# JacekNaruniec/LiveScan3D

Measured on AMD Instinct MI355X. Metric: fused frames/s (N x 512x424 depth -> merged cloud), higher is better.
Workload: dtype f32

## Files before the change

livescan3d_amd/csrc/radial.hip:

```cpp
#include "fusion_shared.hpp"

namespace {


struct RadialParams { float cx, cy, fx, fy, r2, r4, r6, pad; };

__device__ __forceinline__ int f2i_x86(float v)
{
    return (v > -2147483904.0f && v < 2147483648.0f) ? (int)v : (int)0x80000000;
}

__global__ __launch_bounds__(kThreads) void radial_warp_kernel(const FrameDesc *frames, const TileDesc *tiles, const RadialParams *rp,
                                                               const unsigned short *depth, unsigned int *winner, int tiles_per_tick,
                                                               long long tick_pix_stride)
{
    const int tick = blockIdx.x / tiles_per_tick;
    const int tile = blockIdx.x - tick * tiles_per_tick;
    const TileDesc td = tiles[tile];
    const FrameDesc fd = frames[td.frame];
    const RadialParams P = rp[td.frame];
    const unsigned short *dep = depth + tick * tick_pix_stride + fd.depth_off;
    unsigned int *win = winner + tick * tick_pix_stride + fd.depth_off;
    const int p0 = (tile - fd.tile_start) * kTile;
    for (int i = threadIdx.x; i < kTile; i += kThreads) {
        const int p = p0 + i;
        if (p >= fd.npix) break;
        if (dep[p] == 0) continue;
        const int y = p / fd.w, x = p - y * fd.w;
        const float u = ((float)x - P.cx) / P.fx;
        const float v = ((float)y - P.cy) / P.fy;
        const float r = u * u + v * v;
        const float d = 1 - P.r2 * r - P.r4 * r * r - P.r6 * r * r * r;
        const int x_corr = f2i_x86(u * d * P.fx + P.cx);
        const int y_corr = f2i_x86(v * d * P.fy + P.cy);
        if (x_corr >= 0 && y_corr >= 0 && x_corr < fd.w && y_corr < fd.h)
            atomicMax(&win[x_corr + (long long)y_corr * fd.w], (unsigned int)p + 1u);
    }
}

__global__ __launch_bounds__(kThreads) void radial_gather_kernel(const FrameDesc *frames, const TileDesc *tiles, const unsigned short *depth,
                                                                 const unsigned char *rgb, const unsigned int *winner,
                                                                 unsigned short *map_copy, unsigned char *colors_copy, int tiles_per_tick,
                                                                 long long tick_pix_stride)
{
    const int tick = blockIdx.x / tiles_per_tick;
    const int tile = blockIdx.x - tick * tiles_per_tick;
    const TileDesc td = tiles[tile];
    const FrameDesc fd = frames[td.frame];
    const long long fb = tick * tick_pix_stride + fd.depth_off;
    const int p0 = (tile - fd.tile_start) * kTile;
    for (int i = threadIdx.x; i < kTile; i += kThreads) {
        const int p = p0 + i;
        if (p >= fd.npix) break;
        const unsigned int wsrc = winner[fb + p];
        unsigned short d = 0;
        unsigned char c0 = 0, c1 = 0, c2 = 0;
        if (wsrc) {
            const long long s = fb + (long long)(wsrc - 1u);
            d = depth[s];
            c0 = rgb[3 * s]; c1 = rgb[3 * s + 1]; c2 = rgb[3 * s + 2];
        }
        map_copy[fb + p] = d;
        colors_copy[3 * (fb + p)] = c0;
        colors_copy[3 * (fb + p) + 1] = c1;
        colors_copy[3 * (fb + p) + 2] = c2;
    }
}

__global__ __launch_bounds__(kThreads) void radial_cand_fill_kernel(const FrameDesc *frames, const TileDesc *tiles, const RadialParams *rp,
                                                                    unsigned int *count, unsigned int *cand, int *overflow)
{
    const int tile = blockIdx.x;
    const TileDesc td = tiles[tile];
    const FrameDesc fd = frames[td.frame];
    const RadialParams P = rp[td.frame];
    const int p0 = (tile - fd.tile_start) * kTile;
    for (int i = threadIdx.x; i < kTile; i += kThreads) {
        const int p = p0 + i;
        if (p >= fd.npix) break;
        const int y = p / fd.w, x = p - y * fd.w;
        const float u = ((float)x - P.cx) / P.fx;
        const float v = ((float)y - P.cy) / P.fy;
        const float r = u * u + v * v;
        const float d = 1 - P.r2 * r - P.r4 * r * r - P.r6 * r * r * r;
        const int x_corr = f2i_x86(u * d * P.fx + P.cx);
        const int y_corr = f2i_x86(v * d * P.fy + P.cy);
        if (x_corr >= 0 && y_corr >= 0 && x_corr < fd.w && y_corr < fd.h) {
            const long long dst = fd.depth_off + x_corr + (long long)y_corr * fd.w;
            const unsigned int slot = atomicAdd(&count[dst], 1u);
            if (slot < 4) cand[4 * dst + slot] = (unsigned int)p + 1u;
            else atomicOr(overflow, 1);
        }
    }
}

__global__ __launch_bounds__(kThreads) void radial_cand_sort_kernel(uint4 *cand, long long n)
{
    const long long i = (long long)blockIdx.x * kThreads + threadIdx.x;
    if (i >= n) return;
    uint4 c = cand[i];
    auto cswap = [](unsigned int &a, unsigned int &b) { const unsigned int hi = max(a, b), lo = min(a, b); a = hi; b = lo; };
    cswap(c.x, c.y); cswap(c.z, c.w); cswap(c.x, c.z); cswap(c.y, c.w); cswap(c.y, c.z);
    cand[i] = c;
}

template <int ELEM, typename T>
__device__ __forceinline__ void store_tile_run(T *dst, const T *lds, int lead, int n)
{
    static_assert(sizeof(T) == ELEM, "element size");
    const int end = lead + n;
    const int c0 = lead ? 1 : 0, c1 = end >> 4;
    uint4 *g16 = reinterpret_cast<uint4 *>(reinterpret_cast<unsigned char *>(dst) - lead);
    const uint4 *l16 = reinterpret_cast<const uint4 *>(lds);
    for (int j = c0 + (int)threadIdx.x; j < c1; j += kThreads) g16[j] = l16[j];
    const int head = lead ? min(n, 16 - lead) : 0;
    const int tail0 = max(head, 16 * c1 - lead);
    const int t = (int)threadIdx.x * ELEM;
    if (t < head) dst[threadIdx.x] = lds[lead / ELEM + threadIdx.x];
    if (tail0 + t < n) dst[tail0 / ELEM + threadIdx.x] = lds[(lead + tail0) / ELEM + threadIdx.x];
}

constexpr unsigned int kWide = 0xFFFFFFFFu;

__global__ __launch_bounds__(kThreads) void radial_cand_pack_kernel(const FrameDesc *frames, const TileDesc *tiles, const uint4 *cand,
                                                                    unsigned int *ctab)
{
    const int tile = blockIdx.x;
    const TileDesc td = tiles[tile];
    const FrameDesc fd = frames[td.frame];
    const int p0 = (tile - fd.tile_start) * kTile;
    for (int i = threadIdx.x; i < kTile; i += kThreads) {
        const int p = p0 + i;
        if (p >= fd.npix) break;
        const uint4 c = cand[fd.depth_off + p];
        auto enc = [&](unsigned int src, unsigned int &code) {
            code = 0;
            if (!src) return true;
            const int rel = (int)(src - 1u) - p;
            if (rel < -32767 || rel > 32767) return false;
            code = (unsigned int)(rel + 32768);
            return true;
        };
        unsigned int c0, c1;
        const bool ok0 = enc(c.x, c0), ok1 = enc(c.y, c1);
        ctab[fd.depth_off + p] = (ok0 && ok1 && c.z == 0) ? (c0 | (c1 << 16)) : kWide;
    }
}

typedef unsigned int u32_ua __attribute__((aligned(1)));
typedef unsigned short u16_ua __attribute__((aligned(1)));
typedef unsigned long long u64_ua __attribute__((aligned(1)));

struct WarpSrc {
    const unsigned short *depth;
    const unsigned char *rgb;
    const unsigned int *ctab;
    const uint4 *cand;
    long long last_px;
};


constexpr unsigned int kRsrcWord3 = 0x00027000u;
constexpr unsigned int kNowhere = 0xFFFFFFF0u;

template <int K, bool SPEC = false>
__device__ __forceinline__ void gather_batch(const WarpSrc &S, long long fb, long long doff, int npix, int pv, const int (&p)[K], const bool (&in)[K],
                                             unsigned int (&d)[K], unsigned int (&rgb)[K])
{
    (void)pv;
    const __amdgpu_buffer_rsrc_t tab = __builtin_amdgcn_make_buffer_rsrc(const_cast<unsigned int *>(S.ctab + doff), 0, 4 * npix, kRsrcWord3);
    const __amdgpu_buffer_rsrc_t dep = __builtin_amdgcn_make_buffer_rsrc(const_cast<unsigned short *>(S.depth + fb), 0, 2 * npix, kRsrcWord3);
    const __amdgpu_buffer_rsrc_t col = __builtin_amdgcn_make_buffer_rsrc(const_cast<unsigned char *>(S.rgb + 3 * fb), 0, 3 * npix, kRsrcWord3);
    const unsigned int last = (unsigned int)npix - 1u;
    auto colour = [&](unsigned int q, bool real) {
        const unsigned int adj = q == last ? 1u : 0u;
        const unsigned int v = __builtin_amdgcn_raw_buffer_load_b32(col, real ? 3u * q - adj : kNowhere, 0, 0);
        return (v >> (8u * adj)) & 0x00FFFFFFu;
    };
    unsigned int e[K];
#pragma unroll
    for (int k = 0; k < K; k++) e[k] = __builtin_amdgcn_raw_buffer_load_b32(tab, in[k] ? 4u * (unsigned int)p[k] : kNowhere, 0, 0);
    unsigned int s0[K], s1[K], d0[K], d1[K], c0[K];
    bool any_wide = false;
#pragma unroll
    for (int k = 0; k < K; k++) {
        const unsigned int a0 = e[k] & 0xFFFFu, a1 = e[k] >> 16;
        const bool wide = e[k] == kWide;
        any_wide |= wide;
        const bool v0 = a0 != 0 && !wide, v1 = a1 != 0 && !wide;
        s0[k] = (unsigned int)p[k] + a0 - 32768u;
        s1[k] = (unsigned int)p[k] + a1 - 32768u;
        d0[k] = __builtin_amdgcn_raw_buffer_load_b16(dep, v0 ? 2u * s0[k] : kNowhere, 0, 0);
        d1[k] = __builtin_amdgcn_raw_buffer_load_b16(dep, v1 ? 2u * s1[k] : kNowhere, 0, 0);
        if (SPEC) c0[k] = colour(s0[k], v0);
    }
    bool second = false;
#pragma unroll
    for (int k = 0; k < K; k++) {
        const unsigned int src = d0[k] ? s0[k] : s1[k];
        d[k] = d0[k] ? d0[k] : d1[k];
        if (SPEC) {
            rgb[k] = d0[k] ? c0[k] : 0u;
            second |= !d0[k] && d1[k];
        } else {
            rgb[k] = colour(src, d[k] != 0);
        }
    }
    if (SPEC && __any(second)) {
#pragma unroll
        for (int k = 0; k < K; k++) {
            const bool need = !d0[k] && d1[k];
            const unsigned int v = colour(s1[k], need);
            if (need) rgb[k] = v;
        }
    }
    if (__any(any_wide)) {
        const unsigned short *gdep = S.depth + fb;
#pragma unroll
        for (int k = 0; k < K; k++) {
            if (e[k] == kWide) {
                const uint4 c = S.cand[doff + p[k]];
                const unsigned int cs[4] = {c.x, c.y, c.z, c.w};
                int sw = -1;
                unsigned int dd = 0;
#pragma unroll
                for (int j = 0; j < 4; j++) {
                    if (sw < 0 && cs[j]) {
                        const unsigned int v = gdep[cs[j] - 1u];
                        if (v) { sw = (int)(cs[j] - 1u); dd = v; }
                    }
                }
                d[k] = dd;
                rgb[k] = colour((unsigned int)(sw >= 0 ? sw : 0), sw >= 0);
            }
        }
    }
}

__device__ __forceinline__ unsigned int one_pixel_colour(const WarpSrc &S, long long fb, unsigned int depth)
{
    const unsigned char *px = S.rgb + 3 * fb;
    return depth ? ((unsigned int)px[0] | ((unsigned int)px[1] << 8) | ((unsigned int)px[2] << 16)) : 0u;
}

__global__ __launch_bounds__(kThreads) void radial_gather_pack_kernel(const FrameDesc *__restrict__ frames, const TileDesc *__restrict__ tiles,
                                                                      const WarpSrc S, unsigned short *__restrict__ map_copy,
                                                                      unsigned char *__restrict__ colors_copy, int tiles_per_tick, long long tick_pix_stride)
{
    const int tick = blockIdx.x / tiles_per_tick;
    const int tile = blockIdx.x - tick * tiles_per_tick;
    const TileDesc td = tiles[tile];
    const FrameDesc fd = frames[td.frame];
    const long long fb = tick * tick_pix_stride + fd.depth_off;
    const int p0 = (tile - fd.tile_start) * kTile;
    __shared__ alignas(16) unsigned short s_d[kTile + 8];
    __shared__ alignas(16) unsigned char s_c[3 * kTile + 16];
    unsigned short *gd = map_copy + fb + p0;
    unsigned char *gc = colors_copy + 3 * (fb + p0);
    const int lead_d = (int)(reinterpret_cast<uintptr_t>(gd) & 15), lead_c = (int)(reinterpret_cast<uintptr_t>(gc) & 15);
    constexpr int kFly = 4;
    for (int i0 = threadIdx.x; i0 < kTile; i0 += kFly * kThreads) {
        int p[kFly];
        bool in[kFly];
#pragma unroll
        for (int k = 0; k < kFly; k++) {
            p[k] = p0 + i0 + k * kThreads;
            in[k] = i0 + k * kThreads < kTile && p[k] < fd.npix;
        }
        unsigned int d[kFly], c[kFly];
        gather_batch<kFly>(S, fb, fd.depth_off, fd.npix, p0, p, in, d, c);
#pragma unroll
        for (int k = 0; k < kFly; k++) {
            if (!in[k]) continue;
            const int i = i0 + k * kThreads;
            s_d[lead_d / 2 + i] = (unsigned short)d[k];
            unsigned char *c3 = s_c + lead_c + 3 * i;
            c3[0] = (unsigned char)c[k];
            c3[1] = (unsigned char)(c[k] >> 8);
            c3[2] = (unsigned char)(c[k] >> 16);
        }
    }
    if (fd.npix == 1 && threadIdx.x == 0) {
        const unsigned int c1 = one_pixel_colour(S, fb, s_d[lead_d / 2]);
        unsigned char *c3 = s_c + lead_c;
        c3[0] = (unsigned char)c1;
        c3[1] = (unsigned char)(c1 >> 8);
        c3[2] = (unsigned char)(c1 >> 16);
    }
    __syncthreads();
    const int n_px = min(kTile, fd.npix - p0);
    store_tile_run<2>(gd, s_d, lead_d, 2 * n_px);
    store_tile_run<1>(gc, s_c, lead_c, 3 * n_px);
}

constexpr int kRing = 32;

struct RingChunk { unsigned int d[4]; unsigned int c[8]; };

__device__ __forceinline__ void ring_load_chunk(const unsigned short *map, const unsigned char *col, int w, int h, int row, int chunk,
                                                RingChunk &reg)
{
    const bool row_ok = row >= 0 && row < h;
    if ((w & 7) == 0) {
        uint4 dv = make_uint4(0, 0, 0, 0);
// ... 11 lines not shown
            const int b = 3 * j;
            const unsigned int lo = cw[b >> 2], hi = cw[(b >> 2) + 1 < 6 ? (b >> 2) + 1 : 5];
            reg.c[j] = __funnelshift_r(lo, hi, (b & 3) * 8) & 0x00FFFFFFu;
        }
        return;
    }
#pragma unroll
    for (int j = 0; j < 8; j++) {
        const int c0 = chunk * 8 + j;
        unsigned int dv = 0, cv = 0;
        if (row_ok && c0 >= 0 && c0 < w) {
            const long long p = (long long)row * w + c0;
            dv = map[p];
            cv = col[3 * p] | (col[3 * p + 1] << 8) | (col[3 * p + 2] << 16);
        }
        if (j & 1) reg.d[j >> 1] |= dv << 16;
        else reg.d[j >> 1] = dv;
        reg.c[j] = cv;
    }
}

__device__ __forceinline__ void ring_store_chunk(unsigned short *dring_row, unsigned int *cring_row, int chunk, const RingChunk &reg)
{
    const int s0 = (chunk * 8) & (kRing - 1);
    unsigned int *dd = reinterpret_cast<unsigned int *>(dring_row + s0);
#pragma unroll
    for (int j = 0; j < 4; j++) dd[j] = reg.d[j];
#pragma unroll
    for (int j = 0; j < 8; j++) cring_row[s0 + j] = reg.c[j];
}

struct RingFeed {
    int ring, row;
    RingChunk p0, p1;
};

__global__ __launch_bounds__(768) void radial_close_kernel(const FrameDesc *frames, int n_frames, unsigned short *map_copy,
                                                            unsigned char *colors_copy, long long tick_pix_stride)
{
    extern __shared__ unsigned int ring_mem[];
    const int rows = blockDim.x;
    unsigned int *cring = ring_mem;
    unsigned short *dring = reinterpret_cast<unsigned short *>(ring_mem + (rows + 2) * kRing);
    const int tick = blockIdx.x / n_frames;
    const int f = blockIdx.x - tick * n_frames;
    const FrameDesc fd = frames[f];
    const int w = fd.w, h = fd.h;
    unsigned short *map = map_copy + tick * tick_pix_stride + fd.depth_off;
    unsigned char *col = colors_copy + 3 * (tick * tick_pix_stride + fd.depth_off);
    const int r = threadIdx.x;
    for (int band0 = 1; band0 < h - 1; band0 += rows) {
        const int y = band0 + r;
        const bool has_a = y <= h - 1;
        const bool has_b = (r == 0) || (r == rows - 1);
        RingFeed A, B;
        A.ring = r + 1; A.row = y;
        B.ring = r == 0 ? 0 : rows + 1; B.row = r == 0 ? band0 - 1 : y + 1;
        const int x_start = 1 - 2 * r;
        auto top_chunk = [](int x0) { return (x0 + 18) >> 3; };
        __syncthreads();
        {
            const int P = top_chunk(x_start);
            if (has_a) {
                for (int c = P - 3; c <= P; c++) {
                    ring_load_chunk(map, col, w, h, A.row, c, A.p0);
                    ring_store_chunk(dring + A.ring * kRing, cring + A.ring * kRing, c, A.p0);
                }
                ring_load_chunk(map, col, w, h, A.row, P + 1, A.p0);
                ring_load_chunk(map, col, w, h, A.row, P + 2, A.p1);
            }
            if (has_b) {
                for (int c = P - 3; c <= P; c++) {
                    ring_load_chunk(map, col, w, h, B.row, c, B.p0);
                    ring_store_chunk(dring + B.ring * kRing, cring + B.ring * kRing, c, B.p0);
                }
                ring_load_chunk(map, col, w, h, B.row, P + 1, B.p0);
                ring_load_chunk(map, col, w, h, B.row, P + 2, B.p1);
            }
        }
        __syncthreads();
        const unsigned short *d_up = dring + r * kRing, *d_below = dring + (r + 2) * kRing;
        unsigned short *d_mine = dring + (r + 1) * kRing;
        const unsigned int *c_up = cring + r * kRing, *c_below = cring + (r + 2) * kRing;
        unsigned int *c_mine = cring + (r + 1) * kRing;
        const int steps = (w - 2) + 2 * (rows - 1);
        for (int t = 0; t < steps; t++) {
            const int x = x_start + t;
            if (t > 0 && (t & 15) == 0) {
                const int P = top_chunk(x);
                if (has_a) {
                    ring_store_chunk(dring + A.ring * kRing, cring + A.ring * kRing, P - 1, A.p0);
                    ring_store_chunk(dring + A.ring * kRing, cring + A.ring * kRing, P, A.p1);
                    ring_load_chunk(map, col, w, h, A.row, P + 1, A.p0);
                    ring_load_chunk(map, col, w, h, A.row, P + 2, A.p1);
                }
                if (has_b) {
                    ring_store_chunk(dring + B.ring * kRing, cring + B.ring * kRing, P - 1, B.p0);
                    ring_store_chunk(dring + B.ring * kRing, cring + B.ring * kRing, P, B.p1);
                    ring_load_chunk(map, col, w, h, B.row, P + 1, B.p0);
                    ring_load_chunk(map, col, w, h, B.row, P + 2, B.p1);
                }
                __builtin_amdgcn_fence(__ATOMIC_RELEASE, "workgroup", "local");
                __builtin_amdgcn_s_barrier();
                __builtin_amdgcn_fence(__ATOMIC_ACQUIRE, "workgroup", "local");
            }
            if (y < h - 1 && x >= 1 && x < w - 1 && d_mine[x & (kRing - 1)] == 0) {
                const int xm = (x - 1) & (kRing - 1), x0 = x & (kRing - 1), xp = (x + 1) & (kRing - 1);
                const int nb[8] = {d_up[xm], d_up[x0], d_up[xp], d_mine[xm], d_mine[xp], d_below[xm], d_below[x0], d_below[xp]};
                int n = 0, sum = 0, prev_val = -1;
                unsigned int accepted = 0;
#pragma unroll
                for (int i = 0; i < 8; i++) {
                    const bool ok = (nb[i] > 0) & ((prev_val == -1) | (abs(nb[i] - prev_val) < 30));
                    prev_val = ok ? nb[i] : prev_val;
                    n += ok ? 1 : 0;
                    sum += ok ? nb[i] : 0;
                    accepted |= (ok ? 1u : 0u) << i;
                }
                if (n > 4) {
                    const unsigned int nc[8] = {c_up[xm], c_up[x0], c_up[xp], c_mine[xm], c_mine[xp], c_below[xm], c_below[x0], c_below[xp]};
                    int sR = 0, sG = 0, sB = 0;
#pragma unroll
                    for (int i = 0; i < 8; i++) {
                        const unsigned int c = (accepted >> i) & 1u ? nc[i] : 0u;
                        sR += c & 0xFF; sG += (c >> 8) & 0xFF; sB += (c >> 16) & 0xFF;
                    }
                    const float rn = 1.0f / (float)n;
                    auto div_n = [&](int v) {
                        int q = (int)((float)v * rn);
                        const int r = v - q * n;
                        q += r >= n ? 1 : 0;
                        q -= r < 0 ? 1 : 0;
                        return (unsigned int)q;
                    };
                    const unsigned int fd_ = div_n(sum);
                    const unsigned int fR = div_n(sR), fG = div_n(sG), fB = div_n(sB);
                    d_mine[x0] = (unsigned short)fd_;
                    c_mine[x0] = fR | (fG << 8) | (fB << 16);
                    const long long pos = x + (long long)y * w;
                    map[pos] = (unsigned short)fd_;
                    col[pos * 3] = (unsigned char)fR;
                    col[pos * 3 + 1] = (unsigned char)fG;
                    col[pos * 3 + 2] = (unsigned char)fB;
                }
            }
            __builtin_amdgcn_fence(__ATOMIC_RELEASE, "workgroup", "local");
            __builtin_amdgcn_s_barrier();
            __builtin_amdgcn_fence(__ATOMIC_ACQUIRE, "workgroup", "local");
        }
    }
}


__device__ __forceinline__ void accept_chain(const int (&nb)[8], int &n, int &sum, unsigned int &accepted)
{
    n = 0;
    sum = 0;
    accepted = 0;
    int prev_val = -1;
#pragma unroll
    for (int i = 0; i < 8; i++) {
        const bool ok = (nb[i] > 0) & ((prev_val == -1) | (abs(nb[i] - prev_val) < 30));
        prev_val = ok ? nb[i] : prev_val;
        n += ok ? 1 : 0;
        sum += ok ? nb[i] : 0;
        accepted |= (ok ? 1u : 0u) << i;
    }
}

__device__ __forceinline__ unsigned int div_small(int v, int n)
{
    const float rn = 1.0f / (float)n;
    int q = (int)((float)v * rn);
    const int r = v - q * n;
    q += r >= n ? 1 : 0;
    q -= r < 0 ? 1 : 0;
    return (unsigned int)q;
}

__device__ __forceinline__ unsigned int average_colour(const unsigned int (&nc)[8], unsigned int accepted, int n)
{
    int sR = 0, sG = 0, sB = 0;
#pragma unroll
    for (int i = 0; i < 8; i++) {
        const unsigned int c = (accepted >> i) & 1u ? nc[i] : 0u;
        sR += c & 0xFF; sG += (c >> 8) & 0xFF; sB += (c >> 16) & 0xFF;
    }
    return div_small(sR, n) | (div_small(sG, n) << 8) | (div_small(sB, n) << 16);
}

constexpr int kDx[8] = {-1, 0, 1, -1, 1, -1, 0, 1}, kDy[8] = {-1, -1, -1, 0, 0, 1, 1, 1};

__device__ __forceinline__ int wave_reserve(int *counter, int mine)
{
    const int lane = threadIdx.x & 63;
    const int incl = wave_inclusive_scan(mine, lane);
    const int total = __shfl(incl, 63, 64);
    int base = 0;
    if (total > 0) {
        if (lane == 0) base = atomicAdd(counter, total);
        base = __shfl(base, 0, 64);
    }
    return base + incl - mine;
}

constexpr int kCntStride = 32;
#ifndef LSN_BAND_THREADS
#define LSN_BAND_THREADS 256
#endif
constexpr int kBandThreads = LSN_BAND_THREADS;

struct BandDesc { int frame, y0; };

__device__ __forceinline__ long long hole_base_bit(const FrameDesc &fd, int f) { return ((fd.depth_off + 63) & ~63ll) + 64ll * f; }

struct BandArgs {
    const FrameDesc *frames;
    const BandDesc *bands;
    WarpSrc src;
    unsigned short *out_d;
    unsigned char *out_c;
    unsigned char *holes;
    unsigned int *work;
    int *work_cnt;
    int bands_per_tick, n_frames, rows;
    long long tick_pix_stride, holes_tick_bytes;
};

constexpr int kBandList = 8192;

__host__ __device__ inline int band_list_entries(int rows, int w)
{
    const int all = rows * w;
    return all <= kBandList ? all : (kBandList > w ? kBandList : w);
}

__host__ __device__ inline int band_lds_bytes(int rows, int w)
{
    const int band_px = (rows + 2) * w;
    return 16 + ((2 * band_px + 15) & ~15) + 16 + ((3 * band_px + 15) & ~15) + ((2 * band_list_entries(rows, w) + 15) & ~15) + 16;
}

__device__ __forceinline__ void store_band_run(unsigned char *dst, const unsigned char *lds, int n)
{
    const int lead = (int)(reinterpret_cast<uintptr_t>(dst) & 15);
    const int head = lead ? min(n, 16 - lead) : 0;
    const int chunks = (n - head) >> 4;
    const uint4 *l16 = reinterpret_cast<const uint4 *>(lds + head);
    uint4 *g16 = reinterpret_cast<uint4 *>(dst + head);
    for (int j = threadIdx.x; j < chunks; j += kBandThreads) g16[j] = l16[j];
    const int tail0 = head + 16 * chunks;
    if ((int)threadIdx.x < head) dst[threadIdx.x] = lds[threadIdx.x];
    if (tail0 + (int)threadIdx.x < n) dst[tail0 + threadIdx.x] = lds[tail0 + threadIdx.x];
}

__device__ __forceinline__ unsigned int pk_min1(unsigned int x)
{
    unsigned int r;
    asm("v_pk_min_u16 %0, %1, %2" : "=v"(r) : "v"(x), "v"(0x00010001u));
    return r;
}

template <bool GATHER, bool VEC>
__global__ __launch_bounds__(kBandThreads) void radial_band_kernel(const BandArgs a)
{
    extern __shared__ __attribute__((aligned(16))) unsigned char smem[];
    const int tid = threadIdx.x;
    const int tick = blockIdx.x / a.bands_per_tick;
    const int band = blockIdx.x - tick * a.bands_per_tick;
    const BandDesc bd = a.bands[band];
    const FrameDesc fd = a.frames[bd.frame];
    const int w = fd.w, h = fd.h, y0 = bd.y0;
    const int nrows = min(a.rows, h - y0);
    const long long fb = tick * a.tick_pix_stride + fd.depth_off;
    const int tf = tick * a.n_frames + bd.frame;
    const int band_px = (a.rows + 2) * w;
    unsigned short *gd = a.out_d + fb + (long long)y0 * w;
    unsigned char *gc = a.out_c + 3 * (fb + (long long)y0 * w);
    const int lead_d = (int)((reinterpret_cast<uintptr_t>(gd) - 2 * (uintptr_t)w) & 15);
    const int lead_c = (int)((reinterpret_cast<uintptr_t>(gc) - 3 * (uintptr_t)w) & 15);
    const int off_c = 16 + ((2 * band_px + 15) & ~15);
    const int off_l = off_c + 16 + ((3 * band_px + 15) & ~15);
    unsigned short *s_d = reinterpret_cast<unsigned short *>(smem + lead_d);
    unsigned char *s_c = smem + off_c + lead_c;
    unsigned short *s_list = reinterpret_cast<unsigned short *>(smem + off_l);
    const int list_entries = band_list_entries(a.rows, w);
    int *s_n = reinterpret_cast<int *>(smem + off_l + ((2 * list_entries + 15) & ~15));
    const int pl0 = (y0 - 1) * w;
    const int lo = pl0 < 0 ? -pl0 : 0;
    const int hi = min((nrows + 2) * w, fd.npix - pl0);

    if (GATHER) {
#ifndef LSN_BAND_FLY
#define LSN_BAND_FLY 8
#endif
        constexpr int kFly = LSN_BAND_FLY;
        for (int i0 = lo + tid; i0 < hi; i0 += kFly * kBandThreads) {
            int p[kFly];
            bool in[kFly];
#pragma unroll
            for (int k = 0; k < kFly; k++) {
                p[k] = pl0 + i0 + k * kBandThreads;
                in[k] = i0 + k * kBandThreads < hi;
            }
            unsigned int d[kFly], c[kFly];
#ifndef LSN_BAND_SPEC
#define LSN_BAND_SPEC false
#endif
            gather_batch<kFly, LSN_BAND_SPEC>(a.src, fb, fd.depth_off, fd.npix, pl0 + lo, p, in, d, c);
#pragma unroll
            for (int k = 0; k < kFly; k++) {
                if (!in[k]) continue;
                const int i = i0 + k * kBandThreads;
                s_d[i] = (unsigned short)d[k];
                unsigned char *c3 = s_c + 3 * i;
                c3[0] = (unsigned char)c[k];
                c3[1] = (unsigned char)(c[k] >> 8);
                c3[2] = (unsigned char)(c[k] >> 16);
            }
        }
        if (fd.npix == 1 && tid == 0) {
            const unsigned int c1 = one_pixel_colour(a.src, fb, s_d[lo]);
            unsigned char *c3 = s_c + 3 * lo;
            c3[0] = (unsigned char)c1;
            c3[1] = (unsigned char)(c1 >> 8);
            c3[2] = (unsigned char)(c1 >> 16);
        }
    } else if (VEC) {
        const unsigned short *sd = a.src.depth + fb + pl0;
        const unsigned char *sc = a.src.rgb + 3 * (fb + pl0);
        for (int i = lo + 8 * tid; i < hi; i += 8 * kBandThreads) {
            *reinterpret_cast<uint4 *>(s_d + i) = *reinterpret_cast<const uint4 *>(sd + i);
            const uint2 *cp = reinterpret_cast<const uint2 *>(sc + 3 * i);
            uint2 *lp = reinterpret_cast<uint2 *>(s_c + 3 * i);
            const uint2 c0 = cp[0], c1 = cp[1], c2 = cp[2];
            lp[0] = c0; lp[1] = c1; lp[2] = c2;
        }
    } else {
        const unsigned short *sd = a.src.depth + fb + pl0;
        const unsigned char *sc = a.src.rgb + 3 * (fb + pl0);
        for (int i = lo + tid; i < hi; i += kBandThreads) {
            s_d[i] = sd[i];
            s_c[3 * i] = sc[3 * i];
            s_c[3 * i + 1] = sc[3 * i + 1];
            s_c[3 * i + 2] = sc[3 * i + 2];
        }
    }
    __syncthreads();

    store_band_run(reinterpret_cast<unsigned char *>(gd), reinterpret_cast<const unsigned char *>(s_d + w), 2 * nrows * w);
    store_band_run(gc, s_c + 3 * w, 3 * nrows * w);

    const long long hole_bit0 = hole_base_bit(fd, bd.frame);
    unsigned char *holes = a.holes + tick * a.holes_tick_bytes;
    unsigned int *work = a.work + 2 * fb;
    int *work_cnt = a.work_cnt + kCntStride * tf;
    const int rows_per_chunk = max(1, list_entries / w);
    for (int r0 = 0; r0 < nrows; r0 += rows_per_chunk) {
        const int r1 = min(nrows, r0 + rows_per_chunk);
        __syncthreads();
        if (tid == 0) *s_n = 0;
        __syncthreads();
        if (VEC) {
            const int gw = w >> 3, ngroups = (r1 - r0) * gw;
            for (int g0 = 0; g0 < ngroups; g0 += kBandThreads) {
                const int g = g0 + tid;
                unsigned int cb = 0;
                int li = 0;
                if (g < ngroups) {
                    const int r = r0 + g / gw, x0 = (g % gw) << 3, y = y0 + r;
                    li = (r + 1) * w + x0;
                    unsigned int m[3];
#pragma unroll
                    for (int rr = 0; rr < 3; rr++) {
                        const unsigned short *row = s_d + li + (rr - 1) * w;
                        const uint4 c = *reinterpret_cast<const uint4 *>(row);
                        const unsigned int left = x0 > 0 ? row[-1] : 0u, right = x0 + 8 < w ? row[8] : 0u;
                        const unsigned int p0 = pk_min1(c.x) | (pk_min1(c.y) << 2), p1 = pk_min1(c.z) | (pk_min1(c.w) << 2);
                        const unsigned int q0 = (p0 | (p0 >> 15)) & 0xFu, q1 = (p1 | (p1 >> 15)) & 0xFu;
                        m[rr] = (left ? 1u : 0u) | ((q0 | (q1 << 4)) << 1) | (right ? (1u << 9) : 0u);
                    }
                    const unsigned int hb = ~(m[1] >> 1) & 0xFFu;
                    holes[(hole_bit0 + (long long)y * w + x0) >> 3] = (unsigned char)hb;
                    if (y >= 1 && y < h - 1) {
                        const unsigned int n0 = m[0], n1 = m[0] >> 1, n2 = m[0] >> 2, n3 = m[1], n4 = m[1] >> 2, n5 = m[2], n6 = m[2] >> 1, n7 = m[2] >> 2;
                        const unsigned int s1 = n0 ^ n1 ^ n2, c1 = (n0 & n1) | (n2 & (n0 ^ n1));
                        const unsigned int s2 = n5 ^ n6 ^ n7, c2 = (n5 & n6) | (n7 & (n5 ^ n6));
                        const unsigned int s3 = n3 ^ n4, c3 = n3 & n4;
                        const unsigned int t0 = s1 ^ s2 ^ s3, d1 = (s1 & s2) | (s3 & (s1 ^ s2));
                        const unsigned int u0 = c1 ^ c2 ^ c3, e1 = (c1 & c2) | (c3 & (c1 ^ c2));
                        const unsigned int v0 = u0 ^ d1, f1 = u0 & d1;
                        const unsigned int w0 = e1 ^ f1, g1 = e1 & f1;
                        unsigned int inside = 0xFFu;
                        if (x0 == 0) inside &= ~1u;
                        if (x0 + 8 == w) inside &= ~0x80u;
                        cb = (g1 | (w0 & (v0 | t0))) & hb & inside;
                    }
                }
                int slot = wave_reserve(s_n, __popc(cb));
#pragma unroll
                for (int k = 0; k < 8; k++)
                    if ((cb >> k) & 1u) s_list[slot++] = (unsigned short)(li + k);
            }
        } else {
            unsigned int *hw = reinterpret_cast<unsigned int *>(holes);
            const int n_px = (r1 - r0) * w;
            for (int i0 = 0; i0 < n_px; i0 += kBandThreads) {
                const int i = r0 * w + i0 + tid;
                bool cand = false;
                const int li = w + i;
                if (i0 + tid < n_px && s_d[li] == 0) {
                    const int r = i / w, x = i - r * w, y = y0 + r;
                    const long long bit = hole_bit0 + (long long)y * w + x;
                    atomicOr(&hw[bit >> 5], 1u << (bit & 31));
                    if (y >= 1 && y < h - 1 && x >= 1 && x < w - 1) {
                        int nv = 0;
#pragma unroll
                        for (int j = 0; j < 8; j++) nv += s_d[li + kDy[j] * w + kDx[j]] != 0 ? 1 : 0;
                        cand = nv >= 5;
                    }
                }
                const int slot = wave_reserve(s_n, cand ? 1 : 0);
                if (cand) s_list[slot] = (unsigned short)li;
            }
        }
        __syncthreads();
        const int n_cand = *s_n;
        for (int i0 = 0; i0 < n_cand; i0 += kBandThreads) {
            const int i = i0 + tid;
            if (i0 + (tid & ~63) >= n_cand) continue;
            unsigned int succ = 0;
            int x = 0, y = 0;
            if (i < n_cand) {
                const int q = (int)s_list[i];
                int nb[8];
#pragma unroll
                for (int j = 0; j < 8; j++) nb[j] = s_d[q + kDy[j] * w + kDx[j]];
                int n, sum;
                unsigned int accepted;
                accept_chain(nb, n, sum, accepted);
                if (n > 4) {
                    unsigned int nc[8];
#pragma unroll
                    for (int j = 0; j < 8; j++) {
                        const unsigned char *c3 = s_c + 3 * (q + kDy[j] * w + kDx[j]);
                        nc[j] = (accepted >> j) & 1u ? ((unsigned int)c3[0] | ((unsigned int)c3[1] << 8) | ((unsigned int)c3[2] << 16)) : 0u;
                    }
                    const unsigned int rgb = average_colour(nc, accepted, n);
                    const long long pos = fb + pl0 + q;
                    a.out_d[pos] = (unsigned short)div_small(sum, n);
                    a.out_c[3 * pos] = (unsigned char)rgb;
                    a.out_c[3 * pos + 1] = (unsigned char)(rgb >> 8);
                    a.out_c[3 * pos + 2] = (unsigned char)(rgb >> 16);
                    int yl = (int)((float)q * fd.inv_w);
                    x = q - yl * w;
                    if (x < 0) { yl--; x += w; }
                    if (x >= w) { yl++; x -= w; }
                    y = y0 - 1 + yl;
                    const bool below = y + 1 < h - 1;
                    succ = ((nb[4] == 0 && x + 1 < w - 1) ? 1u : 0u) | ((nb[5] == 0 && x - 1 >= 1 && below) ? 2u : 0u) |
                           ((nb[6] == 0 && below) ? 4u : 0u) | ((nb[7] == 0 && x + 1 < w - 1 && below) ? 8u : 0u);
                }
            }
            int slot = wave_reserve(work_cnt, __popc(succ));
#pragma unroll
            for (int sidx = 0; sidx < 4; sidx++) {
                if ((succ >> sidx) & 1u) {
                    const int j = 4 + sidx;
                    if (slot < 2 * fd.npix) work[slot] = (unsigned int)((y + kDy[j]) * w + x + kDx[j]);
                    slot++;
                }
            }
        }
    }
}

#ifndef LSN_FIX_THREADS
#define LSN_FIX_THREADS 256
#endif
constexpr int kFixThreads = LSN_FIX_THREADS;
constexpr int kFixList = 8192;

struct FixArgs {
    const FrameDesc *frames;
    unsigned short *out_d;
    unsigned char *out_c;
    const unsigned char *holes;
    const unsigned int *work;
    int *work_cnt;
    int n_frames, list_cap;
    int n_tf, cnt_index;
    long long tick_pix_stride, holes_tick_bytes;
};

__device__ __forceinline__ bool fix_pixel(unsigned short *out_d, unsigned char *out_c, const unsigned char *holes, long long bit0, int p, int w, int h,
                                          float inv_w, unsigned int &succ, int &x, int &y)
{
    y = (int)((float)p * inv_w);
    x = p - y * w;
    if (x < 0) { y--; x += w; }
    if (x >= w) { y++; x -= w; }
    unsigned int dv[3][3], cv[3][3];
#pragma unroll
    for (int r = 0; r < 3; r++) {
        const int q = p + (r - 1) * w - 1;
        const unsigned int d01 = *reinterpret_cast<const u32_ua *>(out_d + q);
        dv[r][0] = d01 & 0xFFFFu;
        dv[r][1] = d01 >> 16;
        dv[r][2] = out_d[q + 2];
        const unsigned long long c8 = *reinterpret_cast<const u64_ua *>(out_c + 3 * (long long)q);
        cv[r][0] = (unsigned int)c8 & 0xFFFFFFu;
        cv[r][1] = (unsigned int)(c8 >> 24) & 0xFFFFFFu;
        cv[r][2] = (unsigned int)(c8 >> 48) | ((unsigned int)out_c[3 * (long long)q + 8] << 16);
    }
    const long long b1 = bit0 + p + 1, b2 = bit0 + p + w - 1;
    const unsigned int h1 = (holes[b1 >> 3] >> (b1 & 7)) & 1u;
    const unsigned int h2 = ((unsigned int)*reinterpret_cast<const u16_ua *>(holes + (b2 >> 3)) >> (b2 & 7)) & 7u;
    const int nb[8] = {(int)dv[0][0], (int)dv[0][1], (int)dv[0][2], (int)dv[1][0], h1 ? 0 : (int)dv[1][2],
                       (h2 & 1u) ? 0 : (int)dv[2][0], (h2 & 2u) ? 0 : (int)dv[2][1], (h2 & 4u) ? 0 : (int)dv[2][2]};
    const unsigned int nc[8] = {cv[0][0], cv[0][1], cv[0][2], cv[1][0], cv[1][2], cv[2][0], cv[2][1], cv[2][2]};
    const unsigned int od = dv[1][1], orgb = cv[1][1];
    unsigned int nd = 0, nrgb = 0;
    int n, sum;
    unsigned int accepted;
    accept_chain(nb, n, sum, accepted);
    if (n > 4) {
        nd = div_small(sum, n);
        nrgb = average_colour(nc, accepted, n);
    }
    succ = 0;
    if (nd == od && nrgb == orgb) return false;
    out_d[p] = (unsigned short)nd;
    out_c[3 * (long long)p] = (unsigned char)nrgb;
    out_c[3 * (long long)p + 1] = (unsigned char)(nrgb >> 8);
    out_c[3 * (long long)p + 2] = (unsigned char)(nrgb >> 16);
    const bool below = y + 1 < h - 1;
    succ = ((h1 && x + 1 < w - 1) ? 1u : 0u) | (((h2 & 1u) && x - 1 >= 1 && below) ? 2u : 0u) | (((h2 & 2u) && below) ? 4u : 0u) |
           (((h2 & 4u) && x + 1 < w - 1 && below) ? 8u : 0u);
    return true;
}

constexpr int kOverflow = 0x40000000;

__global__ __launch_bounds__(kThreads) void close_fix_round_kernel(const FixArgs a, const unsigned int *list_in, const int *cnt_in, int in_stride,
                                                                   int in_cap_num, int in_cap_den, unsigned int *list_out, int *cnt_out,
                                                                   int out_stride, int out_cap_num, int out_cap_den, int blocks_per_frame)
{
    const int tf = blockIdx.x / blocks_per_frame, b = blockIdx.x - tf * blocks_per_frame;
    const int tick = tf / a.n_frames, f = tf - tick * a.n_frames;
    const FrameDesc fd = a.frames[f];
    const int w = fd.w, h = fd.h;
    const long long fb = tick * a.tick_pix_stride + fd.depth_off;
    const int n_in = cnt_in[kCntStride * tf];
    const int in_cap = (int)((long long)fd.npix * in_cap_num / in_cap_den), out_cap = (int)((long long)fd.npix * out_cap_num / out_cap_den);
    if (n_in > in_cap) {
        if (b == 0 && threadIdx.x == 0) cnt_out[kCntStride * tf] = kOverflow;
        return;
    }
    unsigned short *out_d = a.out_d + fb;
    unsigned char *out_c = a.out_c + 3 * fb;
    const unsigned char *holes = a.holes + tick * a.holes_tick_bytes;
    const long long bit0 = hole_base_bit(fd, f);
    const unsigned int *lin = list_in + in_stride * fb;
    unsigned int *lout = list_out + out_stride * fb;
    for (int i0 = b * kThreads; i0 < n_in; i0 += blocks_per_frame * kThreads) {
        const int i = i0 + (int)threadIdx.x;
        if (i0 + (int)(threadIdx.x & ~63u) >= n_in) continue;
        unsigned int succ = 0;
        int x = 0, y = 0;
        if (i < n_in) fix_pixel(out_d, out_c, holes, bit0, (int)lin[i], w, h, fd.inv_w, succ, x, y);
        int slot = wave_reserve(cnt_out + kCntStride * tf, __popc(succ));
#pragma unroll
        for (int sidx = 0; sidx < 4; sidx++) {
            if ((succ >> sidx) & 1u) {
                const int k = 4 + sidx;
                if (slot < out_cap) lout[slot] = (unsigned int)((y + kDy[k]) * w + x + kDx[k]);
                slot++;
            }
        }
    }
}

__global__ __launch_bounds__(kFixThreads) void close_fix_kernel(const FixArgs a)
{
    __shared__ unsigned int lists[2][kFixList];
    __shared__ int s_n[2];
    __shared__ int s_flag;
    const int tf = blockIdx.x;
    const int tick = tf / a.n_frames, f = tf - tick * a.n_frames;
    const FrameDesc fd = a.frames[f];
    const int w = fd.w, h = fd.h;
    const long long fb = tick * a.tick_pix_stride + fd.depth_off;
    unsigned short *out_d = a.out_d + fb;
    unsigned char *out_c = a.out_c + 3 * fb;
    const unsigned char *holes = a.holes + tick * a.holes_tick_bytes;
    const long long bit0 = hole_base_bit(fd, f);
    int *cnt = a.work_cnt + kCntStride * tf;
    const size_t cnt_step = (size_t)kCntStride * a.n_tf;
    const int n_listed = cnt[a.cnt_index * cnt_step];
    const int n0 = n_listed > 2 * fd.npix ? 0 : n_listed;
    __syncthreads();
    if (threadIdx.x == 0) {
        cnt[0] = cnt[cnt_step] = cnt[2 * cnt_step] = 0;
        s_n[0] = s_n[1] = 0;
        s_flag = 0;
    }
    __syncthreads();
    const unsigned int *glist = a.work + 2 * fb;
    int cur = 0;
    bool sweep = n_listed > 2 * fd.npix;
    for (int round = 0;; round++) {
        const int n_items = round == 0 ? n0 : s_n[cur];
        if (n_items == 0) break;
        for (int i0 = 0; i0 < n_items; i0 += kFixThreads) {
            const int i = i0 + (int)threadIdx.x;
            if (i0 + (int)(threadIdx.x & ~63u) >= n_items) continue;
            unsigned int succ = 0;
            int x = 0, y = 0;
            if (i < n_items) fix_pixel(out_d, out_c, holes, bit0, (int)(round == 0 ? glist[i] : lists[cur][i]), w, h, fd.inv_w, succ, x, y);
            int slot = wave_reserve(&s_n[1 - cur], __popc(succ));
#pragma unroll
            for (int sidx = 0; sidx < 4; sidx++) {
                if ((succ >> sidx) & 1u) {
                    const int k = 4 + sidx;
                    if (slot < a.list_cap) lists[1 - cur][slot] = (unsigned int)((y + kDy[k]) * w + x + kDx[k]);
                    else s_flag = 1;
                    slot++;
                }
            }
        }
        __threadfence_block();
        __syncthreads();
        if (s_flag) { sweep = true; break; }
        cur = 1 - cur;
        if (threadIdx.x == 0) s_n[1 - cur] = 0;
        __syncthreads();
    }
    while (sweep) {
        __syncthreads();
        if (threadIdx.x == 0) s_flag = 0;
        __syncthreads();
        bool changed = false;
        for (int p = w + 1 + (int)threadIdx.x; p < fd.npix - w - 1; p += kFixThreads) {
            const long long b = bit0 + p;
            if (!((holes[b >> 3] >> (b & 7)) & 1u)) continue;
            int x, y;
            {
                y = (int)((float)p * fd.inv_w);
                x = p - y * w;
                if (x < 0) { y--; x += w; }
                if (x >= w) { y++; x -= w; }
            }
            if (x < 1 || x >= w - 1) continue;
            unsigned int succ;
            changed |= fix_pixel(out_d, out_c, holes, bit0, p, w, h, fd.inv_w, succ, x, y);
        }
        if (changed) s_flag = 1;
        __threadfence_block();
        __syncthreads();
        sweep = s_flag != 0;
    }
}

static int make_bands(const LsnFusion *p, int rows, std::vector<BandDesc> &bands)
{
    bands.clear();
    for (int f = 0; f < p->n_maps; f++)
        for (int y0 = 0; y0 < p->h[f]; y0 += rows) bands.push_back(BandDesc{f, y0});
    return (int)bands.size();
}

}

static int radial_correct_on(LsnFusion *p, const float *intr_params, const void *d_depth_in, const void *d_colors_in, void *d_depth, void *d_colors,
                             hipStream_t s);

static int radial_correct(LsnFusion *p, const float *intr_params, const void *d_depth_in, const void *d_colors_in, void *d_depth, void *d_colors,
                          hipStream_t s)
{
    LSN_HIP(hipSetDevice(p->device));
    if (!p->radial_done) LSN_HIP(hipEventCreateWithFlags(&p->radial_done, hipEventDisableTiming));
    if (p->radial_chain_open && p->work_cnt_stream != s) LSN_HIP(hipStreamWaitEvent(s, p->radial_done, 0));
    const int rc = radial_correct_on(p, intr_params, d_depth_in, d_colors_in, d_depth, d_colors, s);
    if (hipEventRecord(p->radial_done, s) == hipSuccess) p->radial_chain_open = true;
    else (void)hipGetLastError();
    p->work_cnt_stream = s;
    return rc;
}

static int radial_correct_on(LsnFusion *p, const float *intr_params, const void *d_depth_in, const void *d_colors_in, void *d_depth, void *d_colors,
                             hipStream_t s)
{
    const bool in_place = d_depth_in == d_depth && d_colors_in == d_colors;
    if (!in_place && (d_depth_in == d_depth || d_colors_in == d_colors)) {
        lsn::set_error("lsnFusionRadialCorrectTo: depth and colours must both be in place or both out of place");
        return -1;
    }
    const size_t npix = (size_t)p->cap * p->n_ticks;
    if (!in_place) {
        auto overlap = [](const void *a, size_t na, const void *b, size_t nb) {
            const uintptr_t x = (uintptr_t)a, y = (uintptr_t)b;
            return x < y + nb && y < x + na;
        };
        if (overlap(d_depth_in, 2 * npix, d_depth, 2 * npix) || overlap(d_colors_in, 3 * npix, d_colors, 3 * npix) ||
            overlap(d_depth_in, 2 * npix, d_colors, 3 * npix) || overlap(d_colors_in, 3 * npix, d_depth, 2 * npix)) {
            lsn::set_error("lsnFusionRadialCorrectTo: the output buffers overlap the input buffers in part (pass the same pointers for an in-place correction)");
            return -1;
        }
    }
    if (p->radial.reserve(sizeof(RadialParams) * p->n_maps)) return -1;
    std::vector<RadialParams> rp(p->n_maps);
    for (int i = 0; i < p->n_maps; i++) {
        const float *ip = intr_params + 7 * i;
        rp[i] = RadialParams{ip[0], ip[1], ip[2], ip[3], ip[4], ip[5], ip[6], 0.0f};
    }
    const int grid = p->tiles_per_tick * p->n_ticks;
    const bool same_intr = p->cand_valid && p->radial_intr.size() == 7 * (size_t)p->n_maps &&
                           memcmp(p->radial_intr.data(), intr_params, sizeof(float) * 7 * p->n_maps) == 0;
    if (!same_intr) {
        LSN_HIP(hipMemcpyAsync(p->radial.p, rp.data(), sizeof(RadialParams) * p->n_maps, hipMemcpyHostToDevice, s));
        LSN_HIP(hipStreamSynchronize(s));
        if (p->cand.reserve(16 * (size_t)p->cap) || p->ctab.reserve(4 * (size_t)p->cap + 16)) return -1;
        unsigned int *count = p->ctab.as<unsigned int>();
        LSN_HIP(hipMemsetAsync(count, 0, 4 * (size_t)p->cap, s));
        LSN_HIP(hipMemsetAsync(p->cand.p, 0, 16 * (size_t)p->cap, s));
        LSN_HIP(hipMemsetAsync(p->misc.as<char>() + 64, 0, sizeof(int), s));
        int *overflow = reinterpret_cast<int *>(p->misc.as<char>() + 64);
        hipLaunchKernelGGL(radial_cand_fill_kernel, dim3(p->tiles_per_tick), dim3(kThreads), 0, s, p->frames.as<FrameDesc>(),
                           p->tile_frame.as<TileDesc>(), p->radial.as<RadialParams>(), count, p->cand.as<unsigned int>(), overflow);
        hipLaunchKernelGGL(radial_cand_sort_kernel, dim3((unsigned)((p->cap + kThreads - 1) / kThreads)), dim3(kThreads), 0, s, p->cand.as<uint4>(),
                           p->cap);
        hipLaunchKernelGGL(radial_cand_pack_kernel, dim3(p->tiles_per_tick), dim3(kThreads), 0, s, p->frames.as<FrameDesc>(),
                           p->tile_frame.as<TileDesc>(), (const uint4 *)p->cand.as<uint4>(), p->ctab.as<unsigned int>());
        int ov = 0;
        LSN_HIP(hipMemcpyAsync(&ov, overflow, sizeof(int), hipMemcpyDeviceToHost, s));
        LSN_HIP(hipStreamSynchronize(s));
        p->cand_overflow = ov != 0;
        p->radial_intr.assign(intr_params, intr_params + 7 * (size_t)p->n_maps);
        p->cand_valid = true;
    }
    const char *force = getenv("LSN_RADIAL_FORCE_ATOMIC");
    const char *close_env = getenv("LSN_RADIAL_CLOSE"), *tiny_env = getenv("LSN_RADIAL_TINY_LISTS");
    const bool atomic_warp = p->cand_overflow || (force && atoi(force) != 0);
    const bool wavefront = close_env && !strcmp(close_env, "wavefront");
    const bool tiny_lists = tiny_env && atoi(tiny_env) != 0;
    const bool vec_ptrs = ((uintptr_t)d_depth & 15) == 0 && ((uintptr_t)d_colors & 7) == 0 && ((uintptr_t)d_depth_in & 15) == 0 &&
                          ((uintptr_t)d_colors_in & 7) == 0 && (p->cap % 8) == 0;
    const bool vec = p->vec_ok && vec_ptrs;
    WarpSrc src;
    src.depth = static_cast<const unsigned short *>(d_depth_in);
    src.rgb = static_cast<const unsigned char *>(d_colors_in);
    src.ctab = p->ctab.as<unsigned int>();
    src.cand = p->cand.as<uint4>();
    src.last_px = (long long)npix - 1;
    const bool scratch = in_place || atomic_warp || wavefront;
    if (scratch) {
        if (p->map_copy.reserve(2 * npix + 16) || p->colors_copy.reserve(3 * npix + 16)) return -1;
        if (!atomic_warp) {
            hipLaunchKernelGGL(radial_gather_pack_kernel, dim3(grid), dim3(kThreads), 0, s, p->frames.as<FrameDesc>(), p->tile_frame.as<TileDesc>(), src,
                               p->map_copy.as<unsigned short>(), p->colors_copy.as<unsigned char>(), p->tiles_per_tick, p->cap);
        } else {
            if (p->winner.reserve(4 * npix)) return -1;
            LSN_HIP(hipMemsetAsync(p->winner.p, 0, 4 * npix, s));
            hipLaunchKernelGGL(radial_warp_kernel, dim3(grid), dim3(kThreads), 0, s, p->frames.as<FrameDesc>(), p->tile_frame.as<TileDesc>(),
                               p->radial.as<RadialParams>(), src.depth, p->winner.as<unsigned int>(), p->tiles_per_tick, p->cap);
            hipLaunchKernelGGL(radial_gather_kernel, dim3(grid), dim3(kThreads), 0, s, p->frames.as<FrameDesc>(), p->tile_frame.as<TileDesc>(),
                               src.depth, src.rgb, (const unsigned int *)p->winner.as<unsigned int>(), p->map_copy.as<unsigned short>(),
                               p->colors_copy.as<unsigned char>(), p->tiles_per_tick, p->cap);
        }
        src.depth = p->map_copy.as<unsigned short>();
        src.rgb = p->colors_copy.as<unsigned char>();
    }
    const int n_tf = p->n_maps * p->n_ticks;
    if (wavefront) {
        int max_h = 1;
        for (int v : p->h) max_h = v > max_h ? v : max_h;
        int rows = max_h - 2 < 64 ? 64 : ((max_h - 2 + 63) / 64) * 64;
        if (rows > 768) rows = 768;
        if ((long long)n_tf > 256 && rows > 256) rows = 256;
        if (const char *env = getenv("LSN_RADIAL_ROWS")) {
            const int v = atoi(env);
            if (v >= 64 && v <= 768 && v % 64 == 0) rows = v;
        }
        const size_t ring_bytes = (sizeof(unsigned int) + sizeof(unsigned short)) * kRing * (rows + 2);
        hipLaunchKernelGGL(radial_close_kernel, dim3((unsigned)n_tf), dim3(rows), ring_bytes, s, p->frames.as<FrameDesc>(), p->n_maps,
                           p->map_copy.as<unsigned short>(), p->colors_copy.as<unsigned char>(), p->cap);
        LSN_HIP(hipGetLastError());
        LSN_HIP(hipMemcpyAsync(d_depth, p->map_copy.p, 2 * npix, hipMemcpyDeviceToDevice, s));
        LSN_HIP(hipMemcpyAsync(d_colors, p->colors_copy.p, 3 * npix, hipMemcpyDeviceToDevice, s));
// ... 147 lines not shown
```

Before: 220,000.

## Streamline neighbour accept, magic-number division and aligned RGB gathers in fill kernels

Replaces the per-pixel accept chain with an unsigned range-check formulation, and replaces the float-reciprocal divisions with multiply-shift magic constants valid for n in 5..8. It also computes the colour average with packed SWAR sums. Shared-memory and global RGB/depth neighbour reads become aligned word loads recombined with alignbit instead of byte loads. The close_fix loop uses a triple-buffered counter so one barrier per round can be dropped. The risks are subtle correctness issues around the counter reuse and the aligned over-reads past buffer edges.

```diff
diff --git a/livescan3d_amd/csrc/radial.hip b/livescan3d_amd/csrc/radial.hip
--- a/livescan3d_amd/csrc/radial.hip
+++ b/livescan3d_amd/csrc/radial.hip
@@ -1,4 +1,5 @@
 #include "fusion_shared.hpp"
+#include "radial_eval.hpp"
 
 namespace {
 
@@ -146,10 +147,6 @@
         ctab[fd.depth_off + p] = (ok0 && ok1 && c.z == 0) ? (c0 | (c1 << 16)) : kWide;
     }
 }
-
-typedef unsigned int u32_ua __attribute__((aligned(1)));
-typedef unsigned short u16_ua __attribute__((aligned(1)));
-typedef unsigned long long u64_ua __attribute__((aligned(1)));
 
 struct WarpSrc {
     const unsigned short *depth;
@@ -467,43 +464,6 @@
 }
 
 
-__device__ __forceinline__ void accept_chain(const int (&nb)[8], int &n, int &sum, unsigned int &accepted)
-{
-    n = 0;
-    sum = 0;
-    accepted = 0;
-    int prev_val = -1;
-#pragma unroll
-    for (int i = 0; i < 8; i++) {
-        const bool ok = (nb[i] > 0) & ((prev_val == -1) | (abs(nb[i] - prev_val) < 30));
-        prev_val = ok ? nb[i] : prev_val;
-        n += ok ? 1 : 0;
-        sum += ok ? nb[i] : 0;
-        accepted |= (ok ? 1u : 0u) << i;
-    }
-}
-
-__device__ __forceinline__ unsigned int div_small(int v, int n)
-{
-    const float rn = 1.0f / (float)n;
-    int q = (int)((float)v * rn);
-    const int r = v - q * n;
-    q += r >= n ? 1 : 0;
-    q -= r < 0 ? 1 : 0;
-    return (unsigned int)q;
-}
-
-__device__ __forceinline__ unsigned int average_colour(const unsigned int (&nc)[8], unsigned int accepted, int n)
-{
-    int sR = 0, sG = 0, sB = 0;
-#pragma unroll
-    for (int i = 0; i < 8; i++) {
-        const unsigned int c = (accepted >> i) & 1u ? nc[i] : 0u;
-        sR += c & 0xFF; sG += (c >> 8) & 0xFF; sB += (c >> 16) & 0xFF;
-    }
-    return div_small(sR, n) | (div_small(sG, n) << 8) | (div_small(sB, n) << 16);
-}
-
 constexpr int kDx[8] = {-1, 0, 1, -1, 1, -1, 0, 1}, kDy[8] = {-1, -1, -1, 0, 0, 1, 1, 1};
 
 __device__ __forceinline__ int wave_reserve(int *counter, int mine)
@@ -567,6 +527,26 @@
     const int tail0 = head + 16 * chunks;
     if ((int)threadIdx.x < head) dst[threadIdx.x] = lds[threadIdx.x];
     if (tail0 + (int)threadIdx.x < n) dst[tail0 + threadIdx.x] = lds[tail0 + threadIdx.x];
+}
+
+__device__ __forceinline__ void put_rgb(unsigned char *c3, unsigned int c)
+{
+    volatile __attribute__((address_space(3))) unsigned char *v = (volatile __attribute__((address_space(3))) unsigned char *)c3;
+    v[0] = (unsigned char)c;
+    v[1] = (unsigned char)(c >> 8);
+    v[2] = (unsigned char)(c >> 16);
+}
+
+__device__ __forceinline__ void get_rgb3(const unsigned char *s_c, int q, unsigned int &c0, unsigned int &c1, unsigned int &c2)
+{
+    const unsigned char *b = s_c + 3 * (q - 1);
+    const unsigned int mis = (unsigned int)reinterpret_cast<uintptr_t>(b) & 3u, sh = 8u * mis;
+    const unsigned int *a = reinterpret_cast<const unsigned int *>(b - mis);
+    const unsigned int x0 = a[0], x1 = a[1], x2 = a[2];
+    const unsigned int y0 = __builtin_amdgcn_alignbit(x1, x0, sh), y1 = __builtin_amdgcn_alignbit(x2, x1, sh), y2 = x2 >> sh;
+    c0 = y0 & 0xFFFFFFu;
+    c1 = __builtin_amdgcn_alignbit(y1, y0, 24) & 0xFFFFFFu;
+    c2 = __builtin_amdgcn_alignbit(y2, y1, 16) & 0xFFFFFFu;
 }
 
 __device__ __forceinline__ unsigned int pk_min1(unsigned int x)
@@ -628,19 +608,11 @@
                 if (!in[k]) continue;
                 const int i = i0 + k * kBandThreads;
                 s_d[i] = (unsigned short)d[k];
-                unsigned char *c3 = s_c + 3 * i;
-                c3[0] = (unsigned char)c[k];
-                c3[1] = (unsigned char)(c[k] >> 8);
-                c3[2] = (unsigned char)(c[k] >> 16);
-            }
-        }
-        if (fd.npix == 1 && tid == 0) {
-            const unsigned int c1 = one_pixel_colour(a.src, fb, s_d[lo]);
-            unsigned char *c3 = s_c + 3 * lo;
-            c3[0] = (unsigned char)c1;
-            c3[1] = (unsigned char)(c1 >> 8);
-            c3[2] = (unsigned char)(c1 >> 16);
-        }
+                put_rgb(s_c + 3 * i, c[k]);
+            }
+        }
+        if (fd.npix == 1 && tid == 0)
+            put_rgb(s_c + 3 * lo, one_pixel_colour(a.src, fb, s_d[lo]));
     } else if (VEC) {
         const unsigned short *sd = a.src.depth + fb + pl0;
         const unsigned char *sc = a.src.rgb + 3 * (fb + pl0);
@@ -752,18 +724,16 @@
 #pragma unroll
                 for (int j = 0; j < 8; j++) nb[j] = s_d[q + kDy[j] * w + kDx[j]];
                 int n, sum;
-                unsigned int accepted;
-                accept_chain(nb, n, sum, accepted);
+                const unsigned int accepted = lsn_eval::accept_mask(nb, n, sum);
                 if (n > 4) {
-                    unsigned int nc[8];
-#pragma unroll
-                    for (int j = 0; j < 8; j++) {
-                        const unsigned char *c3 = s_c + 3 * (q + kDy[j] * w + kDx[j]);
-                        nc[j] = (accepted >> j) & 1u ? ((unsigned int)c3[0] | ((unsigned int)c3[1] << 8) | ((unsigned int)c3[2] << 16)) : 0u;
-                    }
-                    const unsigned int rgb = average_colour(nc, accepted, n);
+                    unsigned int nc[8], own;
+                    get_rgb3(s_c, q - w, nc[0], nc[1], nc[2]);
+                    get_rgb3(s_c, q, nc[3], own, nc[4]);
+                    get_rgb3(s_c, q + w, nc[5], nc[6], nc[7]);
+                    (void)own;
+                    const unsigned int rgb = lsn_eval::average_rgb(nc, accepted, n);
                     const long long pos = fb + pl0 + q;
-                    a.out_d[pos] = (unsigned short)div_small(sum, n);
+                    a.out_d[pos] = (unsigned short)lsn_eval::div_by_n((unsigned int)sum, lsn_eval::magic_of(n));
                     a.out_c[3 * pos] = (unsigned char)rgb;
                     a.out_c[3 * pos + 1] = (unsigned char)(rgb >> 8);
                     a.out_c[3 * pos + 2] = (unsigned char)(rgb >> 16);
@@ -808,6 +778,9 @@
     long long tick_pix_stride, holes_tick_bytes;
 };
 
+typedef unsigned long long u64_a4 __attribute__((aligned(4)));
+typedef unsigned int u32x3_a4 __attribute__((ext_vector_type(3), aligned(4)));
+
 __device__ __forceinline__ bool fix_pixel(unsigned short *out_d, unsigned char *out_c, const unsigned char *holes, long long bit0, int p, int w, int h,
                                           float inv_w, unsigned int &succ, int &x, int &y)
 {
@@ -815,33 +788,49 @@
     x = p - y * w;
     if (x < 0) { y--; x += w; }
     if (x >= w) { y++; x -= w; }
-    unsigned int dv[3][3], cv[3][3];
+    unsigned long long d4[3];
+    u32x3_a4 c12[3];
+    unsigned int dsh[3], csh[3];
 #pragma unroll
     for (int r = 0; r < 3; r++) {
         const int q = p + (r - 1) * w - 1;
-        const unsigned int d01 = *reinterpret_cast<const u32_ua *>(out_d + q);
+        const unsigned short *dq = out_d + q;
+        const unsigned char *cq = out_c + 3 * (long long)q;
+        const unsigned int dmis = (unsigned int)reinterpret_cast<uintptr_t>(dq) & 3u, cmis = (unsigned int)reinterpret_cast<uintptr_t>(cq) & 3u;
+        d4[r] = *reinterpret_cast<const u64_a4 *>(dq - (dmis >> 1));
+        c12[r] = *reinterpret_cast<const u32x3_a4 *>(cq - cmis);
+        dsh[r] = dmis * 8u;
+        csh[r] = cmis * 8u;
+    }
+    const long long b1 = bit0 + p + 1, b2 = bit0 + p + w - 1;
+    const unsigned int h1 = (holes[b1 >> 3] >> (b1 & 7)) & 1u;
+    const unsigned long long hw = *reinterpret_cast<const u64_a4 *>(holes + 4 * (b2 >> 5));
+#pragma unroll
+    for (int r = 0; r < 3; r++) asm volatile("" : "+v"(c12[r]));
+    unsigned int dv[3][3], cv[3][3];
+#pragma unroll
+    for (int r = 0; r < 3; r++) {
+        const unsigned int d01 = __builtin_amdgcn_alignbit((unsigned int)(d4[r] >> 32), (unsigned int)d4[r], dsh[r]);
         dv[r][0] = d01 & 0xFFFFu;
         dv[r][1] = d01 >> 16;
-        dv[r][2] = out_d[q + 2];
-        const unsigned long long c8 = *reinterpret_cast<const u64_ua *>(out_c + 3 * (long long)q);
-        cv[r][0] = (unsigned int)c8 & 0xFFFFFFu;
-        cv[r][1] = (unsigned int)(c8 >> 24) & 0xFFFFFFu;
-        cv[r][2] = (unsigned int)(c8 >> 48) | ((unsigned int)out_c[3 * (long long)q + 8] << 16);
-    }
-    const long long b1 = bit0 + p + 1, b2 = bit0 + p + w - 1;
-    const unsigned int h1 = (holes[b1 >> 3] >> (b1 & 7)) & 1u;
-    const unsigned int h2 = ((unsigned int)*reinterpret_cast<const u16_ua *>(holes + (b2 >> 3)) >> (b2 & 7)) & 7u;
+        dv[r][2] = ((unsigned int)(d4[r] >> 32) >> dsh[r]) & 0xFFFFu;
+        const u32x3_a4 c = c12[r];
+        const unsigned int y0 = __builtin_amdgcn_alignbit(c.y, c.x, csh[r]), y1 = __builtin_amdgcn_alignbit(c.z, c.y, csh[r]), y2 = c.z >> csh[r];
+        cv[r][0] = y0 & 0xFFFFFFu;
+        cv[r][1] = __builtin_amdgcn_alignbit(y1, y0, 24) & 0xFFFFFFu;
+        cv[r][2] = __builtin_amdgcn_alignbit(y2, y1, 16) & 0xFFFFFFu;
+    }
+    const unsigned int h2 = __builtin_amdgcn_alignbit((unsigned int)(hw >> 32), (unsigned int)hw, (unsigned int)(b2 & 31)) & 7u;
     const int nb[8] = {(int)dv[0][0], (int)dv[0][1], (int)dv[0][2], (int)dv[1][0], h1 ? 0 : (int)dv[1][2],
                        (h2 & 1u) ? 0 : (int)dv[2][0], (h2 & 2u) ? 0 : (int)dv[2][1], (h2 & 4u) ? 0 : (int)dv[2][2]};
     const unsigned int nc[8] = {cv[0][0], cv[0][1], cv[0][2], cv[1][0], cv[1][2], cv[2][0], cv[2][1], cv[2][2]};
     const unsigned int od = dv[1][1], orgb = cv[1][1];
     unsigned int nd = 0, nrgb = 0;
     int n, sum;
-    unsigned int accepted;
-    accept_chain(nb, n, sum, accepted);
+    const unsigned int accepted = lsn_eval::accept_mask(nb, n, sum);
     if (n > 4) {
-        nd = div_small(sum, n);
-        nrgb = average_colour(nc, accepted, n);
+        nd = lsn_eval::div_by_n((unsigned int)sum, lsn_eval::magic_of(n));
+        nrgb = lsn_eval::average_rgb(nc, accepted, n);
     }
     succ = 0;
     if (nd == od && nrgb == orgb) return false;
@@ -899,7 +888,7 @@
 __global__ __launch_bounds__(kFixThreads) void close_fix_kernel(const FixArgs a)
 {
     __shared__ unsigned int lists[2][kFixList];
-    __shared__ int s_n[2];
+    __shared__ int s_n[3];
     __shared__ int s_flag;
     const int tf = blockIdx.x;
     const int tick = tf / a.n_frames, f = tf - tick * a.n_frames;
@@ -917,23 +906,24 @@
     __syncthreads();
     if (threadIdx.x == 0) {
         cnt[0] = cnt[cnt_step] = cnt[2 * cnt_step] = 0;
-        s_n[0] = s_n[1] = 0;
+        s_n[0] = s_n[1] = s_n[2] = 0;
         s_flag = 0;
     }
     __syncthreads();
     const unsigned int *glist = a.work + 2 * fb;
-    int cur = 0;
     bool sweep = n_listed > 2 * fd.npix;
     for (int round = 0;; round++) {
-        const int n_items = round == 0 ? n0 : s_n[cur];
+        const int cur = round & 1, c_in = round % 3, c_out = (round + 1) % 3;
+        const int n_items = round == 0 ? n0 : s_n[c_in];
         if (n_items == 0) break;
+        if (threadIdx.x == 0) s_n[(round + 2) % 3] = 0;
         for (int i0 = 0; i0 < n_items; i0 += kFixThreads) {
             const int i = i0 + (int)threadIdx.x;
             if (i0 + (int)(threadIdx.x & ~63u) >= n_items) continue;
             unsigned int succ = 0;
             int x = 0, y = 0;
             if (i < n_items) fix_pixel(out_d, out_c, holes, bit0, (int)(round == 0 ? glist[i] : lists[cur][i]), w, h, fd.inv_w, succ, x, y);
-            int slot = wave_reserve(&s_n[1 - cur], __popc(succ));
+            int slot = wave_reserve(&s_n[c_out], __popc(succ));
 #pragma unroll
             for (int sidx = 0; sidx < 4; sidx++) {
                 if ((succ >> sidx) & 1u) {
@@ -947,9 +937,6 @@
         __threadfence_block();
         __syncthreads();
         if (s_flag) { sweep = true; break; }
-        cur = 1 - cur;
-        if (threadIdx.x == 0) s_n[1 - cur] = 0;
-        __syncthreads();
     }
     while (sweep) {
         __syncthreads();
diff --git a/livescan3d_amd/csrc/radial_eval.hpp b/livescan3d_amd/csrc/radial_eval.hpp
--- /dev/null
+++ b/livescan3d_amd/csrc/radial_eval.hpp
@@ -0,0 +1,55 @@
+#pragma once
+
+#if defined(__HIPCC__)
+#define LSN_EVAL_FN __host__ __device__ __forceinline__
+#else
+#define LSN_EVAL_FN inline
+#endif
+
+namespace lsn_eval {
+
+LSN_EVAL_FN unsigned int accept_mask(const int (&nb)[8], int &n, int &sum)
+{
+    unsigned int lo = 1u, rg = 0xFFFFFFFEu, m = 0u;
+    int s = 0;
+#pragma unroll
+    for (int i = 0; i < 8; i++) {
+        const unsigned int v = (unsigned int)nb[i];
+        const unsigned int lo_i = (v > 30u ? v : 30u) - 29u;
+        const unsigned int rg_i = v + 29u - lo_i;
+        const bool ok = v - lo <= rg;
+        lo = ok ? lo_i : lo;
+        rg = ok ? rg_i : rg;
+        s += ok ? (int)v : 0;
+        m |= ok ? (1u << i) : 0u;
+    }
+    n = __builtin_popcount(m);
+    sum = s;
+    return m;
+}
+
+LSN_EVAL_FN unsigned int div_by_n(unsigned int v, unsigned int magic)
+{
+    return (unsigned int)(((unsigned long long)v * magic) >> 34);
+}
+
+LSN_EVAL_FN unsigned int magic_of(int n)
+{
+    return n == 5 ? 3435973837u : n == 6 ? 2863311531u : n == 7 ? 2454267027u : 2147483648u;
+}
+
+LSN_EVAL_FN unsigned int average_rgb(const unsigned int (&nc)[8], unsigned int accepted, int n)
+{
+    unsigned int all = 0u, rb = 0u;
+#pragma unroll
+    for (int i = 0; i < 8; i++) {
+        const unsigned int c = (accepted >> i) & 1u ? nc[i] : 0u;
+        all += c;
+        rb += c & 0x00FF00FFu;
+    }
+    const unsigned int mg = magic_of(n);
+    const unsigned int r = div_by_n(rb & 0xFFFFu, mg), b = div_by_n(rb >> 16, mg), g = div_by_n((all - rb) >> 8, mg);
+    return r | (g << 8) | (b << 16);
+}
+
+}
```

After: 219,200 (median of 6 runs). No clear change (-0.4%).
